# jiaw-z/DKT-Stereo

Measured on AMD Instinct MI355X. Metric: stereo pairs/sec at 736x1248 D=192, 32 iters (RAFT-Stereo test_mode forward), higher is better.
Workload: dtype f32 io/accumulate; convolution products = 3x fp16-split MFMA (22-bit operands); lookup / correlation exact fp32

## Files before the change

dkt_stereo_amd/csrc/conv_ws.h:

```cpp

static constexpr int conv_ws_group_first(int g) { return g < 5 ? g : g == 5 ? 5 : g < 10 ? g + 1 : g == 10 ? 11 : g + 2; }
static constexpr int conv_ws_group_units(int g) { return (g == 5 || g == 10) ? 2 : 1; }

static constexpr int conv_ws_rows_fed(int r, int nf) {
    int n = 0;
    for (int dy = 0; dy < 3; ++dy) n += (r - dy >= 0 && r - dy < nf) ? 1 : 0;
    return n;
}

typedef _Float16 ws_h2 __attribute__((ext_vector_type(2)));
typedef float ws_f2 __attribute__((ext_vector_type(2)));
__device__ __forceinline__ unsigned ws_bits(ws_h2 h) {
    union { ws_h2 h; unsigned u; } v;
    v.h = h;
    return v.u;
}

template <int NRM, int EPI>
__global__ __launch_bounds__(256, 1) void conv64_ws_kernel(ConvArgs a) {
    constexpr int HALO = 1;
    constexpr int NF = 4, WN = 2;
    constexpr int TR = NF * WN;
    constexpr int PR = TR + 2, PC = 34, NPP = PR * PC;
    constexpr int PITCH = 12;
    constexpr int PLANE = NPP * PITCH;
    constexpr int STAGE = 2 * PLANE;
    constexpr int NCH = 4;
    constexpr int NG = 16;
    constexpr int RB = 4;
    extern __shared__ __attribute__((aligned(16))) unsigned lds[];

    const int tid = threadIdx.x;
    const int lane = tid & 63, wave = tid >> 6;
    const int wm = wave & 1, wn = wave >> 1;
    const int li = lane & 31, kg = lane >> 5;
    const long HW = (long)a.H * a.W;
    const int tiles_h = a.tiles_xy / a.tiles_w;

    const int nblk = (int)gridDim.x;
    const int lb = (nblk % 8 == 0) ? ((int)blockIdx.x % 8) * (nblk / 8) + (int)blockIdx.x / 8 : (int)blockIdx.x;
    auto decode = [&](int t, int &th0, int &tw0, int &tb) {
        const int xy = t % a.tiles_xy;
        tb = t / a.tiles_xy;
        th0 = (xy % tiles_h) * TR;
        tw0 = (xy / tiles_h) * 32;
    };
    int h0, w0, b;
    int tile = lb;
    decode(tile, h0, w0, b);

    f16x8 Ahi[NCH * 9], Alo[NCH * 9];
    auto load_weights = [&]() {
        const long wlane = (long)(wm * 32 + li) * 16 + kg * 8;
#pragma unroll
        for (int c = 0; c < NCH; ++c)
#pragma unroll
            for (int tap = 0; tap < 9; ++tap) {
                const long off = ((long)tap * NCH + c) * (64 * 16) + wlane;
                Ahi[c * 9 + tap] = *(const f16x8 *)(a.whi + off);
                Alo[c * 9 + tap] = *(const f16x8 *)(a.wlo + off);
            }
#pragma unroll
        for (int i = 0; i < NCH * 9; ++i) {
            if (i < 24) {
                asm volatile("" : "+a"(Ahi[i]));
                asm volatile("" : "+a"(Alo[i]));
            } else {
                asm volatile("" : "+v"(Ahi[i]));
                asm volatile("" : "+v"(Alo[i]));
            }
        }
    };

    constexpr int SG = 2, PG = 2;
    constexpr int SIT = (NPP + 64 * PG - 1) / (64 * PG);
    constexpr int NSL = SIT * 4;
    const int swave = __builtin_amdgcn_readfirstlane(wave) % SG;
    const int spgrp = __builtin_amdgcn_readfirstlane(wave) / SG;
    unsigned spix[SIT];
    float sscale[SIT];
    float sreg[SIT][8];
    unsigned shw[SIT][4], slw[SIT][4];
    __amdgpu_buffer_rsrc_t srsrc;
    const unsigned plane_bytes = (unsigned)HW * 4u;
    float nmean[NRM ? 8 : 1], ninv[NRM ? 8 : 1];
    auto stage_tile = [&](int th0, int tw0) {
#pragma unroll
        for (int it = 0; it < SIT; ++it) {
            const int pp = lane + 64 * (it * PG + spgrp);
            const int pr = pp / PC, pc = pp - pr * PC;
            const int ih = th0 - HALO + pr, iw = tw0 - HALO + pc;
            const bool ok = pp < NPP && ih >= 0 && ih < a.H && iw >= 0 && iw < a.W;
            sscale[it] = ok ? a.in_scale : 0.0f;
            spix[it] = ok ? (unsigned)(ih * a.W + iw) * 4u : 0u;
        }
    };
    auto stage_select = [&](int tb, int chunk) {
        const int cb = chunk * 16 + 8 * swave;
        const float *sbase = a.src[0] + (long)tb * a.src_bs[0] + (long)cb * HW;
        const unsigned lo32 = __builtin_amdgcn_readfirstlane((unsigned)(size_t)sbase);
        const unsigned hi32 = __builtin_amdgcn_readfirstlane((unsigned)((size_t)sbase >> 32));
        srsrc = __builtin_amdgcn_make_buffer_rsrc((void *)(((size_t)hi32 << 32) | lo32), 0, (int)(8u * plane_bytes), 0x00020000);
        if (NRM) {
            const float *np = (const float *)(lds + 2 * STAGE + 8) + 2 * (tb * 64 + cb);
#pragma unroll
            for (int j = 0; j < (NRM ? 8 : 1); ++j) {
                nmean[j] = __int_as_float(__builtin_amdgcn_readfirstlane(__float_as_int(np[2 * j])));
                ninv[j] = __int_as_float(__builtin_amdgcn_readfirstlane(__float_as_int(np[2 * j + 1])));
            }
        }
    };
    auto stage_load = [&](int k0, int k1) {
#pragma unroll
        for (int k = k0; k < k1; ++k) {
            if (k >= NSL) break;
            const int it = k >> 2, q = k & 3;
#pragma unroll
            for (int jj = 0; jj < 2; ++jj) {
                const int j = 2 * q + jj;
                sreg[it][j] = __uint_as_float(__builtin_amdgcn_raw_buffer_load_b32(srsrc, spix[it], j * plane_bytes, 0));
            }
        }
    };
    auto stage_store = [&](unsigned *buf, int k0, int k1) {
#pragma unroll
        for (int k = k0; k < k1; ++k) {
            if (k >= NSL) break;
            const int it = k >> 2, q = k & 3;
            float u0 = sreg[it][2 * q], u1 = sreg[it][2 * q + 1];
            if (NRM) {
                u0 = dkt_relu(__fmul_rn(__fsub_rn(u0, nmean[(2 * q) % (NRM ? 8 : 1)]), ninv[(2 * q) % (NRM ? 8 : 1)]));
                u1 = dkt_relu(__fmul_rn(__fsub_rn(u1, nmean[(2 * q + 1) % (NRM ? 8 : 1)]), ninv[(2 * q + 1) % (NRM ? 8 : 1)]));
            }
            const ws_f2 xv = {u0 * sscale[it], u1 * sscale[it]};
            const ws_h2 hv = __builtin_convertvector(xv, ws_h2);
            const ws_f2 rv = {xv[0] - (float)hv[0], xv[1] - (float)hv[1]};
            const ws_h2 lv = __builtin_convertvector(rv, ws_h2);
            shw[it][q] = ws_bits(hv);
            slw[it][q] = ws_bits(lv);
            if (q == 3) {
                const int pp = lane + 64 * (it * PG + spgrp);
                unsigned *dst = pp < NPP ? buf + pp * PITCH + 4 * swave : lds + 2 * STAGE;
                *(uint4 *)dst = make_uint4(shw[it][0], shw[it][1], shw[it][2], shw[it][3]);
                *(uint4 *)(dst + (pp < NPP ? PLANE : 4)) = make_uint4(slw[it][0], slw[it][1], slw[it][2], slw[it][3]);
            }
        }
    };

    f32x16 acc[NF];
    auto zero_acc = [&]() {
#pragma unroll
        for (int n = 0; n < NF; ++n)
#pragma unroll
            for (int r = 0; r < 16; ++r) acc[n][r] = 0.0f;
    };
    zero_acc();

    f16x8 Bhi[RB], Blo[RB];
    auto loadB = [&](int slot, const unsigned *buf, int s) {
        const int dx = s / (NF + 2), r = s % (NF + 2);
        const int pp = (wn * NF + r) * PC + li + dx;
        const unsigned *pb = buf + pp * PITCH + kg * 4;
        Bhi[slot] = *(const f16x8 *)pb;
        Blo[slot] = *(const f16x8 *)(pb + PLANE);
    };
    auto mma = [&](const int c, const int s) {
        const int dx = s / (NF + 2), r = s % (NF + 2);
        const int slot = s % RB;
#pragma unroll
        for (int dy = 0; dy < 3; ++dy) {
            const int n = r - dy;
            if (n >= 0 && n < NF)
                acc[n] = __builtin_amdgcn_mfma_f32_32x32x16_f16(Ahi[c * 9 + dy * 3 + dx], Bhi[slot], acc[n], 0, 0, 0);
        }
#pragma unroll
        for (int dy = 0; dy < 3; ++dy) {
            const int n = r - dy;
            if (n >= 0 && n < NF)
                acc[n] = __builtin_amdgcn_mfma_f32_32x32x16_f16(Alo[c * 9 + dy * 3 + dx], Bhi[slot], acc[n], 0, 0, 0);
        }
#pragma unroll
        for (int dy = 0; dy < 3; ++dy) {
            const int n = r - dy;
            if (n >= 0 && n < NF)
                acc[n] = __builtin_amdgcn_mfma_f32_32x32x16_f16(Ahi[c * 9 + dy * 3 + dx], Blo[slot], acc[n], 0, 0, 0);
        }
    };

    auto mma_group = [&](const int c, const int g) {
#pragma unroll
        for (int pass = 0; pass < 3; ++pass)
#pragma unroll
            for (int u = conv_ws_group_first(g); u < conv_ws_group_first(g) + conv_ws_group_units(g); ++u) {
                const int dx = u / (NF + 2), r = u % (NF + 2);
#pragma unroll
                for (int dy = 0; dy < 3; ++dy) {
                    const int n = r - dy;
                    if (n >= 0 && n < NF) {
                        const int t = c * 9 + dy * 3 + dx;
                        acc[n] = __builtin_amdgcn_mfma_f32_32x32x16_f16(pass == 1 ? Alo[t] : Ahi[t], pass == 2 ? Blo[u % RB] : Bhi[u % RB],
                                                                        acc[n], 0, 0, 0);
                    }
                }
            }
    };

    auto wave_rsrc = [&](const float *base) {
        const unsigned lo32 = __builtin_amdgcn_readfirstlane((unsigned)(size_t)base);
        const unsigned hi32 = __builtin_amdgcn_readfirstlane((unsigned)((size_t)base >> 32));
        return __builtin_amdgcn_make_buffer_rsrc((void *)(((size_t)hi32 << 32) | lo32), 0, (int)(32u * plane_bytes), 0x00020000);
    };
    auto epilogue = [&]() {
        const int co_lane = wm * 32 + 4 * kg;
        float bv[16];
#pragma unroll
        for (int r = 0; r < 16; ++r) bv[r] = a.bias ? a.bias[co_lane + (r & 3) + 8 * (r >> 2)] : 0.0f;
        const auto orsrc = wave_rsrc(a.out + (long)b * a.out_bs + (long)(wm * 32) * HW);
        auto row_off = [&](int n, bool &ok) {
            const int oh = h0 + wn * NF + n, ow = w0 + li;
            ok = oh < a.H && ow < a.W;
            return ok ? (unsigned)(4 * kg) * plane_bytes + (unsigned)(oh * a.W + ow) * 4u : 0x80000000u;
        };
        if (EPI == 3) {
            const auto crsrc = wave_rsrc(a.e_c0 + (long)b * a.e_c0_bs + (long)(wm * 32) * HW);
            float gc[2][16];
            unsigned vo[NF];
            auto request = [&](int n) {
#pragma unroll
                for (int r = 0; r < 16; ++r)
                    gc[n & 1][r] = __uint_as_float(__builtin_amdgcn_raw_buffer_load_b32(crsrc, vo[n], ((r & 3) + 8 * (r >> 2)) * plane_bytes, 0));
            };
#pragma unroll
            for (int n = 0; n < NF; ++n) {
                bool ok;
                vo[n] = row_off(n, ok);
            }
            request(0);
            request(1);
#pragma unroll
            for (int n = 0; n < NF; ++n) {
                float o[16];
#pragma unroll
                for (int r = 0; r < 16; ++r) {
                    const float v = acc[n][r] * a.out_scale + bv[r];
                    o[r] = dkt_relu(__fadd_rn(gc[n & 1][r], a.relu ? dkt_relu(v) : v));
                }
                __builtin_amdgcn_sched_barrier(0);
                if (n + 2 < NF) request(n + 2);
                __builtin_amdgcn_sched_barrier(0);
#pragma unroll
                for (int r = 0; r < 16; ++r)
                    __builtin_amdgcn_raw_buffer_store_b32(__float_as_uint(o[r]), orsrc, vo[n], ((r & 3) + 8 * (r >> 2)) * plane_bytes, 0);
                __builtin_amdgcn_sched_barrier(0);
            }
            return;
        }
        float s1[EPI == 1 ? 16 : 1], s2[EPI == 1 ? 16 : 1];
#pragma unroll
        for (int i = 0; i < (EPI == 1 ? 16 : 1); ++i) s1[i] = s2[i] = 0.0f;
#pragma unroll
        for (int n = 0; n < NF; ++n) {
            bool ok;
            const unsigned vo = row_off(n, ok);
#pragma unroll
            for (int r = 0; r < 16; ++r) {
                float v = acc[n][r] * a.out_scale + bv[r];
                if (a.relu) v = dkt_relu(v);
                __builtin_amdgcn_raw_buffer_store_b32(__float_as_uint(v), orsrc, vo, ((r & 3) + 8 * (r >> 2)) * plane_bytes, 0);
                if (EPI == 1) {
                    v = ok ? v : 0.0f;
                    s1[r] = __fadd_rn(s1[r], v);
                    s2[r] = __fadd_rn(s2[r], __fmul_rn(v, v));
                }
            }
            __builtin_amdgcn_sched_barrier(0);
        }
        if (EPI == 1) {
#pragma unroll
            for (int i = 0; i < 16; ++i) {
                s1[i] = __fadd_rn(s1[i], __shfl_xor(s1[i], 16, 32));
                s2[i] = __fadd_rn(s2[i], __shfl_xor(s2[i], 16, 32));
            }
#pragma unroll
            for (int d = 8; d >= 1; d >>= 1) {
                const bool up = (li & d) != 0;
#pragma unroll
                for (int j = 0; j < d; ++j) {
                    const float k1 = up ? s1[j + d] : s1[j], g1 = up ? s1[j] : s1[j + d];
                    const float k2 = up ? s2[j + d] : s2[j], g2 = up ? s2[j] : s2[j + d];
                    s1[j] = __fadd_rn(k1, __shfl_xor(g1, d, 32));
                    s2[j] = __fadd_rn(k2, __shfl_xor(g2, d, 32));
                }
            }
            const int vi = li & 15;
            const int co = co_lane + (vi & 3) + 8 * (vi >> 2);
            const long e = (long)((h0 / TR) * a.tiles_w + w0 / 32) * WN + wn;
            if (li < 16) {
                float *p = a.stats_ws + (((long)b * a.tiles_xy * WN + e) * 64 + co) * 2;
                p[0] = s1[0];
                p[1] = s2[0];
            }
        }
    };

    if (NRM) {
        float *np = (float *)(lds + 2 * STAGE + 8);
        for (int i = tid; i < a.n_co * 128; i += 256) np[i] = a.in_norm[i];
        __syncthreads();
    }
    stage_tile(h0, w0);
    stage_select(b, 0);
    stage_load(0, NSL);
    stage_store(lds, 0, NSL);
    __builtin_amdgcn_sched_barrier(0);
    load_weights();
    __syncthreads();
    loadB(0, lds, 0);
    loadB(1, lds, 1);
    for (;;) {
        const int tn = tile + nblk;
        const bool have_next = tn < a.total_tiles;
        int nh0 = h0, nw0 = w0, nb = b;
        if (have_next) decode(tn, nh0, nw0, nb);
#pragma unroll
        for (int c = 0; c < NCH; ++c) {
            const unsigned *cur = lds + (c & 1) * STAGE;
            unsigned *nxt = lds + ((c + 1) & 1) * STAGE;
            if (c + 1 < NCH) {
                stage_select(b, c + 1);
            } else {
                stage_select(nb, 0);
                stage_tile(nh0, nw0);
            }
#pragma unroll
            for (int g = 0; g < NG; ++g) {
                if (g + 2 < NG) {
#pragma unroll
                    for (int u = conv_ws_group_first(g + 2); u < conv_ws_group_first(g + 2) + conv_ws_group_units(g + 2); ++u)
                        loadB(u % RB, cur, u);
                }
                if (g < 6) stage_load(2 * g, 2 * g + 2);
                else if (g == 9) stage_store(nxt, 0, 1);
                else if (g >= 10 && g < 15) stage_store(nxt, 2 * (g - 10) + 1, 2 * (g - 10) + 3);
                else if (g == 15) stage_store(nxt, 11, 12);
                mma_group(c, g);
                if (conv_ws_group_units(g) == 1 && conv_ws_rows_fed(conv_ws_group_first(g) % (NF + 2), NF) == 1) {
                    __builtin_amdgcn_sched_group_barrier(0x008, 3, 0);
                } else {
                    int nm = 0;
#pragma unroll
                    for (int u = conv_ws_group_first(g); u < conv_ws_group_first(g) + conv_ws_group_units(g); ++u)
                        nm += 3 * conv_ws_rows_fed(u % (NF + 2), NF);
#pragma unroll
                    for (int i = 0; i < nm; ++i) {
                        __builtin_amdgcn_sched_group_barrier(0x008, 1, 0);
                        __builtin_amdgcn_sched_group_barrier(0x320, 1, 0);
                        if (g >= 9) __builtin_amdgcn_sched_group_barrier(0x002, 4, 0);
                        else __builtin_amdgcn_sched_group_barrier(0x002, 2, 0);
                    }
                }
                __builtin_amdgcn_sched_barrier(0);
            }
            asm volatile("s_waitcnt lgkmcnt(0)" ::: "memory");
            __builtin_amdgcn_s_barrier();
            if (c + 1 < NCH) {
                loadB(0, nxt, 0);
                loadB(1, nxt, 1);
            }
        }
        epilogue();
        if (!have_next) break;
        tile = tn; h0 = nh0; w0 = nw0; b = nb;
        loadB(0, lds, 0);
        loadB(1, lds, 1);
        zero_acc();
    }
}

static int launch_conv_ws(ConvArgs a, int B, hipStream_t st) {
    constexpr int STAGE = 10 * 34 * 12 * 2;
    const size_t lds = ((size_t)2 * STAGE + 8) * sizeof(unsigned) + (a.in_norm ? (size_t)B * 512 : 0);
    static int ready[64] = {0};
    int dev = 0;
    (void)hipGetDevice(&dev);
    const int epi = a.epi == 3 ? 3 : (a.stats_ws ? 1 : 0);
    const void *kern = nullptr;
    if (a.in_norm) kern = epi == 3 ? (const void *)conv64_ws_kernel<1, 3> : epi == 1 ? (const void *)conv64_ws_kernel<1, 1> : (const void *)conv64_ws_kernel<1, 0>;
    else kern = epi == 3 ? (const void *)conv64_ws_kernel<0, 3> : epi == 1 ? (const void *)conv64_ws_kernel<0, 1> : (const void *)conv64_ws_kernel<0, 0>;
    if (!ready[dev & 63]) {
        const void *all[6] = {(const void *)conv64_ws_kernel<0, 0>, (const void *)conv64_ws_kernel<0, 1>, (const void *)conv64_ws_kernel<0, 3>,
                              (const void *)conv64_ws_kernel<1, 0>, (const void *)conv64_ws_kernel<1, 1>, (const void *)conv64_ws_kernel<1, 3>};
        for (int i = 0; i < 6; ++i) {
            hipError_t e = hipFuncSetAttribute(all[i], hipFuncAttributeMaxDynamicSharedMemorySize, (int)(((size_t)2 * STAGE + 8) * sizeof(unsigned)) + 64 * 512);
            if (e != hipSuccess) return (int)e;
        }
        int cus = 0;
        if (hipDeviceGetAttribute(&cus, hipDeviceAttributeMultiprocessorCount, dev) != hipSuccess || cus < 1) cus = 256;
        ready[dev & 63] = cus;
    }
    a.tiles_xy = a.tiles_w * ((a.H + 7) / 8);
    a.n_co = B;
    const long total = (long)a.tiles_xy * B;
    if (total > 0x7fffffffL) return DKT_E_SHAPE;
    a.total_tiles = (int)total;
    const long cap = ready[dev & 63];
    long nblk = total > cap ? cap : total;
    if (total > cap) {
        const long rounds = (total + cap - 1) / cap;
        const long need = ((total + rounds - 1) / rounds + 7) & ~7L;
        if (need < nblk) nblk = need;
    }
    void *params[1] = {(void *)&a};
    (void)hipLaunchKernel(kern, dim3((unsigned)nblk), dim3(256), params, lds, st);
    int rc = dkt_launch_status();
    if (rc == DKT_OK && a.stats_ws)
        rc = conv_stats_reduce(a.stats_ws, a.stats_part, B, a.Cout, (long)a.tiles_xy * 2, (long)a.H * a.W, a.out, a.out_bs, st);
    return rc;
}
```

Before: 33.11.

## Use 16x16x32 MFMA with swapped operands and vectorized epilogue stores in conv_ws

Adds a 16x16x32 MFMA variant of the 64-channel 3x3 conv kernel, used by default for the non-stats epilogues. It swaps operand roles so pixels feed the A slot and weights the B slot, and restructures the LDS staging layout into octet planes processed in two column phases per chunk. Because each lane now holds consecutive output pixels, the epilogue can emit 128-bit buffer stores and loads for residual input when the tile is fully in bounds. The aim is to cut strided scalar stores and possibly gain MFMA throughput. The cost is more complex scheduling, a new LDS layout and extra phase loops.

Result: no change. 33.10 (-0.0%).

```diff
diff --git a/dkt_stereo_amd/csrc/conv_ws.h b/dkt_stereo_amd/csrc/conv_ws.h
--- a/dkt_stereo_amd/csrc/conv_ws.h
+++ b/dkt_stereo_amd/csrc/conv_ws.h
@@ -1,3 +1,10 @@
+
+#ifdef CONV_WS_MFMA
+static constexpr int conv_ws_mfma(int, int) { return CONV_WS_MFMA; }
+#else
+static constexpr int conv_ws_mfma(int , int epi) { return epi == 1 ? 32 : 16; }
+#endif
+static constexpr int conv_ws_stage_words(int ms) { return ms == 16 ? 2 * 4 * 1408 : 2 * (10 * 34 + 1) * 12; }
 
 static constexpr int conv_ws_group_first(int g) { return g < 5 ? g : g == 5 ? 5 : g < 10 ? g + 1 : g == 10 ? 11 : g + 2; }
 static constexpr int conv_ws_group_units(int g) { return (g == 5 || g == 10) ? 2 : 1; }
@@ -10,6 +17,8 @@
 
 typedef _Float16 ws_h2 __attribute__((ext_vector_type(2)));
 typedef float ws_f2 __attribute__((ext_vector_type(2)));
+typedef float ws_f4 __attribute__((ext_vector_type(4)));
+typedef unsigned ws_u4 __attribute__((ext_vector_type(4)));
 __device__ __forceinline__ unsigned ws_bits(ws_h2 h) {
     union { ws_h2 h; unsigned u; } v;
     v.h = h;
@@ -18,22 +27,26 @@
 
 template <int NRM, int EPI>
 __global__ __launch_bounds__(256, 1) void conv64_ws_kernel(ConvArgs a) {
+    constexpr int MS = conv_ws_mfma(NRM, EPI);
     constexpr int HALO = 1;
     constexpr int NF = 4, WN = 2;
     constexpr int TR = NF * WN;
     constexpr int PR = TR + 2, PC = 34, NPP = PR * PC;
-    constexpr int PITCH = 12;
-    constexpr int PLANE = NPP * PITCH;
-    constexpr int STAGE = 2 * PLANE;
-    constexpr int NCH = 4;
+    constexpr int PITCH = MS == 16 ? 4 : 12;
+    constexpr int OCT = MS == 16 ? 1408 : 4;
+    constexpr int PLANE = MS == 16 ? 4 * OCT : (NPP + 1) * PITCH;
+    constexpr int STAGE = conv_ws_stage_words(MS);
+    constexpr int NCH = MS == 16 ? 2 : 4;
+    constexpr int NPH = MS == 16 ? 2 : 1;
     constexpr int NG = 16;
     constexpr int RB = 4;
+    constexpr int LSH = MS == 16 ? 4 : 5;
     extern __shared__ __attribute__((aligned(16))) unsigned lds[];
 
     const int tid = threadIdx.x;
     const int lane = tid & 63, wave = tid >> 6;
     const int wm = wave & 1, wn = wave >> 1;
-    const int li = lane & 31, kg = lane >> 5;
+    const int li = lane & (MS - 1), kg = lane >> LSH;
     const long HW = (long)a.H * a.W;
     const int tiles_h = a.tiles_xy / a.tiles_w;
 
@@ -49,25 +62,25 @@
     int tile = lb;
     decode(tile, h0, w0, b);
 
-    f16x8 Ahi[NCH * 9], Alo[NCH * 9];
+    f16x8 Whi[36], Wlo[36];
     auto load_weights = [&]() {
-        const long wlane = (long)(wm * 32 + li) * 16 + kg * 8;
-#pragma unroll
-        for (int c = 0; c < NCH; ++c)
-#pragma unroll
-            for (int tap = 0; tap < 9; ++tap) {
-                const long off = ((long)tap * NCH + c) * (64 * 16) + wlane;
-                Ahi[c * 9 + tap] = *(const f16x8 *)(a.whi + off);
-                Alo[c * 9 + tap] = *(const f16x8 *)(a.wlo + off);
-            }
-#pragma unroll
-        for (int i = 0; i < NCH * 9; ++i) {
+#pragma unroll
+        for (int i = 0; i < 36; ++i) {
+            const int h = MS == 16 ? i & 1 : 0, ct = MS == 16 ? i >> 1 : i;
+            const int c = ct / 9, tap = ct % 9;
+            const int ci16 = MS == 16 ? 2 * c + (kg >> 1) : c;
+            const long off = ((long)tap * 4 + ci16) * (64 * 16) + (long)(wm * 32 + 16 * h + li) * 16 + (MS == 16 ? kg & 1 : kg) * 8;
+            Whi[i] = *(const f16x8 *)(a.whi + off);
+            Wlo[i] = *(const f16x8 *)(a.wlo + off);
+        }
+#pragma unroll
+        for (int i = 0; i < 36; ++i) {
             if (i < 24) {
-                asm volatile("" : "+a"(Ahi[i]));
-                asm volatile("" : "+a"(Alo[i]));
+                asm volatile("" : "+a"(Whi[i]));
+                asm volatile("" : "+a"(Wlo[i]));
             } else {
-                asm volatile("" : "+v"(Ahi[i]));
-                asm volatile("" : "+v"(Alo[i]));
+                asm volatile("" : "+v"(Whi[i]));
+                asm volatile("" : "+v"(Wlo[i]));
             }
         }
     };
@@ -78,6 +91,12 @@
     const int swave = __builtin_amdgcn_readfirstlane(wave) % SG;
     const int spgrp = __builtin_amdgcn_readfirstlane(wave) / SG;
     unsigned spix[SIT];
+    unsigned sdst[SIT];
+#pragma unroll
+    for (int it = 0; it < SIT; ++it) {
+        const int pp = lane + 64 * (it * PG + spgrp);
+        sdst[it] = (unsigned)((pp < NPP ? pp : NPP) * PITCH);
+    }
     float sscale[SIT];
     float sreg[SIT][8];
     unsigned shw[SIT][4], slw[SIT][4];
@@ -95,14 +114,14 @@
             spix[it] = ok ? (unsigned)(ih * a.W + iw) * 4u : 0u;
         }
     };
-    auto stage_select = [&](int tb, int chunk) {
-        const int cb = chunk * 16 + 8 * swave;
+    auto stage_select = [&](int tb, int grp) {
+        const int cb = grp * 16 + 8 * swave;
         const float *sbase = a.src[0] + (long)tb * a.src_bs[0] + (long)cb * HW;
         const unsigned lo32 = __builtin_amdgcn_readfirstlane((unsigned)(size_t)sbase);
         const unsigned hi32 = __builtin_amdgcn_readfirstlane((unsigned)((size_t)sbase >> 32));
         srsrc = __builtin_amdgcn_make_buffer_rsrc((void *)(((size_t)hi32 << 32) | lo32), 0, (int)(8u * plane_bytes), 0x00020000);
         if (NRM) {
-            const float *np = (const float *)(lds + 2 * STAGE + 8) + 2 * (tb * 64 + cb);
+            const float *np = (const float *)(lds + 2 * STAGE) + 2 * (tb * 64 + cb);
 #pragma unroll
             for (int j = 0; j < (NRM ? 8 : 1); ++j) {
                 nmean[j] = __int_as_float(__builtin_amdgcn_readfirstlane(__float_as_int(np[2 * j])));
@@ -122,7 +141,7 @@
             }
         }
     };
-    auto stage_store = [&](unsigned *buf, int k0, int k1) {
+    auto stage_store = [&](unsigned *buf, const int grp, int k0, int k1) {
 #pragma unroll
         for (int k = k0; k < k1; ++k) {
             if (k >= NSL) break;
@@ -139,55 +158,43 @@
             shw[it][q] = ws_bits(hv);
             slw[it][q] = ws_bits(lv);
             if (q == 3) {
-                const int pp = lane + 64 * (it * PG + spgrp);
-                unsigned *dst = pp < NPP ? buf + pp * PITCH + 4 * swave : lds + 2 * STAGE;
+                const int oct = MS == 16 ? 2 * (grp & 1) + swave : swave;
+                unsigned *dst = buf + sdst[it] + oct * OCT;
                 *(uint4 *)dst = make_uint4(shw[it][0], shw[it][1], shw[it][2], shw[it][3]);
-                *(uint4 *)(dst + (pp < NPP ? PLANE : 4)) = make_uint4(slw[it][0], slw[it][1], slw[it][2], slw[it][3]);
-            }
-        }
-    };
-
-    f32x16 acc[NF];
+                *(uint4 *)(dst + PLANE) = make_uint4(slw[it][0], slw[it][1], slw[it][2], slw[it][3]);
+            }
+        }
+    };
+
+    ws_f4 acc16[MS == 16 ? 2 : 1][NF][2];
+    f32x16 acc32[NF];
     auto zero_acc = [&]() {
 #pragma unroll
-        for (int n = 0; n < NF; ++n)
-#pragma unroll
-            for (int r = 0; r < 16; ++r) acc[n][r] = 0.0f;
+        for (int n = 0; n < NF; ++n) {
+            if (MS == 16) {
+#pragma unroll
+                for (int i = 0; i < 4; ++i)
+#pragma unroll
+                    for (int r = 0; r < 4; ++r) acc16[(i >> 1) % (MS == 16 ? 2 : 1)][n][i & 1][r] = 0.0f;
+            } else {
+#pragma unroll
+                for (int r = 0; r < 16; ++r) acc32[n][r] = 0.0f;
+            }
+        }
     };
     zero_acc();
 
-    f16x8 Bhi[RB], Blo[RB];
-    auto loadB = [&](int slot, const unsigned *buf, int s) {
-        const int dx = s / (NF + 2), r = s % (NF + 2);
-        const int pp = (wn * NF + r) * PC + li + dx;
-        const unsigned *pb = buf + pp * PITCH + kg * 4;
-        Bhi[slot] = *(const f16x8 *)pb;
-        Blo[slot] = *(const f16x8 *)(pb + PLANE);
-    };
-    auto mma = [&](const int c, const int s) {
-        const int dx = s / (NF + 2), r = s % (NF + 2);
-        const int slot = s % RB;
-#pragma unroll
-        for (int dy = 0; dy < 3; ++dy) {
-            const int n = r - dy;
-            if (n >= 0 && n < NF)
-                acc[n] = __builtin_amdgcn_mfma_f32_32x32x16_f16(Ahi[c * 9 + dy * 3 + dx], Bhi[slot], acc[n], 0, 0, 0);
-        }
-#pragma unroll
-        for (int dy = 0; dy < 3; ++dy) {
-            const int n = r - dy;
-            if (n >= 0 && n < NF)
-                acc[n] = __builtin_amdgcn_mfma_f32_32x32x16_f16(Alo[c * 9 + dy * 3 + dx], Bhi[slot], acc[n], 0, 0, 0);
-        }
-#pragma unroll
-        for (int dy = 0; dy < 3; ++dy) {
-            const int n = r - dy;
-            if (n >= 0 && n < NF)
-                acc[n] = __builtin_amdgcn_mfma_f32_32x32x16_f16(Ahi[c * 9 + dy * 3 + dx], Blo[slot], acc[n], 0, 0, 0);
-        }
-    };
-
-    auto mma_group = [&](const int c, const int g) {
+    f16x8 Fhi[RB], Flo[RB];
+    const unsigned rbase = (unsigned)((wn * NF * PC + li) * PITCH + kg * OCT);
+    auto loadF = [&](int slot, const unsigned *buf, const int ph, const int u) {
+        const int dx = u / (NF + 2), r = u % (NF + 2);
+        const int pc = r * PC + 16 * ph + dx;
+        const unsigned *pb = buf + rbase + pc * PITCH;
+        Fhi[slot] = *(const f16x8 *)pb;
+        Flo[slot] = *(const f16x8 *)(pb + PLANE);
+    };
+
+    auto mma_group = [&](const int c, const int ph, const int g) {
 #pragma unroll
         for (int pass = 0; pass < 3; ++pass)
 #pragma unroll
@@ -198,8 +205,15 @@
                     const int n = r - dy;
                     if (n >= 0 && n < NF) {
                         const int t = c * 9 + dy * 3 + dx;
-                        acc[n] = __builtin_amdgcn_mfma_f32_32x32x16_f16(pass == 1 ? Alo[t] : Ahi[t], pass == 2 ? Blo[u % RB] : Bhi[u % RB],
-                                                                        acc[n], 0, 0, 0);
+                        const f16x8 x = pass == 2 ? Flo[u % RB] : Fhi[u % RB];
+                        if (MS == 16) {
+#pragma unroll
+                            for (int h = 0; h < 2; ++h)
+                                acc16[h % (MS == 16 ? 2 : 1)][n][ph] = __builtin_amdgcn_mfma_f32_16x16x32_f16(
+                                    x, pass == 1 ? Wlo[(2 * t + h) % 36] : Whi[(2 * t + h) % 36], acc16[h % (MS == 16 ? 2 : 1)][n][ph], 0, 0, 0);
+                        } else {
+                            acc32[n] = __builtin_amdgcn_mfma_f32_32x32x16_f16(x, pass == 1 ? Wlo[t % 36] : Whi[t % 36], acc32[n], 0, 0, 0);
+                        }
                     }
                 }
             }
@@ -210,113 +224,148 @@
         const unsigned hi32 = __builtin_amdgcn_readfirstlane((unsigned)((size_t)base >> 32));
         return __builtin_amdgcn_make_buffer_rsrc((void *)(((size_t)hi32 << 32) | lo32), 0, (int)(32u * plane_bytes), 0x00020000);
     };
-    auto epilogue = [&]() {
-        const int co_lane = wm * 32 + 4 * kg;
-        float bv[16];
-#pragma unroll
-        for (int r = 0; r < 16; ++r) bv[r] = a.bias ? a.bias[co_lane + (r & 3) + 8 * (r >> 2)] : 0.0f;
+    auto epilogue = [&](auto wide_c) {
+        constexpr bool WIDE = decltype(wide_c)::value;
+        constexpr int NQ = 4, NH = MS == 16 ? 2 : 1;
+        auto qh = [](int q) { return MS == 16 ? q >> 1 : 0; };
+        auto qpx = [](int q) { return MS == 16 ? 16 * (q & 1) : 8 * q; };
+        auto val = [&](int n, int q, int j) { return MS == 16 ? acc16[qh(q) % NH][n][q & 1][j] : acc32[n][4 * q + j]; };
+        int lane_e = lane;
+        asm volatile("" : "+v"(lane_e));
+        const int li = lane_e & (MS - 1), kg = lane_e >> LSH;
+        const int co_lane = wm * 32 + li;
+        float bv[NH];
+#pragma unroll
+        for (int h = 0; h < NH; ++h) bv[h] = a.bias ? a.bias[co_lane + 16 * h] : 0.0f;
         const auto orsrc = wave_rsrc(a.out + (long)b * a.out_bs + (long)(wm * 32) * HW);
-        auto row_off = [&](int n, bool &ok) {
-            const int oh = h0 + wn * NF + n, ow = w0 + li;
-            ok = oh < a.H && ow < a.W;
-            return ok ? (unsigned)(4 * kg) * plane_bytes + (unsigned)(oh * a.W + ow) * 4u : 0x80000000u;
+        unsigned vo[NF];
+        const int ow = w0 + 4 * kg;
+#pragma unroll
+        for (int n = 0; n < NF; ++n) {
+            const int oh = h0 + wn * NF + n;
+            vo[n] = oh < a.H ? (unsigned)li * plane_bytes + (unsigned)(oh * a.W + ow) * 4u : 0x80000000u;
+        }
+        auto q_soff = [&](int q) { return (unsigned)(16 * qh(q)) * plane_bytes + (unsigned)(qpx(q) * 4); };
+        const int left = a.W - ow;
+        auto q_voff = [&](int n, int q, int j) {
+            int lf = left;
+            if (!WIDE) asm volatile("" : "+v"(lf));
+            return qpx(q) + j < lf ? vo[n] : 0x80000000u;
+        };
+        auto store_run = [&](int n, int q, const float (&o)[4]) {
+            if (WIDE) {
+                const ws_u4 v = {__float_as_uint(o[0]), __float_as_uint(o[1]), __float_as_uint(o[2]), __float_as_uint(o[3])};
+                __builtin_amdgcn_raw_buffer_store_b128(v, orsrc, q_voff(n, q, 0), q_soff(q), 0);
+            } else {
+#pragma unroll
+                for (int j = 0; j < 4; ++j)
+                    __builtin_amdgcn_raw_buffer_store_b32(__float_as_uint(o[j]), orsrc, q_voff(n, q, j), q_soff(q) + 4 * j, 0);
+            }
         };
         if (EPI == 3) {
             const auto crsrc = wave_rsrc(a.e_c0 + (long)b * a.e_c0_bs + (long)(wm * 32) * HW);
-            float gc[2][16];
-            unsigned vo[NF];
+            float gc[2][NQ][4];
             auto request = [&](int n) {
 #pragma unroll
-                for (int r = 0; r < 16; ++r)
-                    gc[n & 1][r] = __uint_as_float(__builtin_amdgcn_raw_buffer_load_b32(crsrc, vo[n], ((r & 3) + 8 * (r >> 2)) * plane_bytes, 0));
+                for (int q = 0; q < NQ; ++q) {
+                    if (WIDE) {
+                        const ws_u4 v = __builtin_amdgcn_raw_buffer_load_b128(crsrc, q_voff(n, q, 0), q_soff(q), 0);
+#pragma unroll
+                        for (int j = 0; j < 4; ++j) gc[n & 1][q][j] = __uint_as_float(v[j]);
+                    } else {
+#pragma unroll
+                        for (int j = 0; j < 4; ++j)
+                            gc[n & 1][q][j] = __uint_as_float(__builtin_amdgcn_raw_buffer_load_b32(crsrc, q_voff(n, q, j), q_soff(q) + 4 * j, 0));
+                    }
+                }
             };
-#pragma unroll
-            for (int n = 0; n < NF; ++n) {
-                bool ok;
-                vo[n] = row_off(n, ok);
-            }
             request(0);
             request(1);
 #pragma unroll
             for (int n = 0; n < NF; ++n) {
-                float o[16];
-#pragma unroll
-                for (int r = 0; r < 16; ++r) {
-                    const float v = acc[n][r] * a.out_scale + bv[r];
-                    o[r] = dkt_relu(__fadd_rn(gc[n & 1][r], a.relu ? dkt_relu(v) : v));
-                }
+                float o[NQ][4];
+#pragma unroll
+                for (int q = 0; q < NQ; ++q)
+#pragma unroll
+                    for (int j = 0; j < 4; ++j) {
+                        const float v = val(n, q, j) * a.out_scale + bv[qh(q) % NH];
+                        o[q][j] = dkt_relu(__fadd_rn(gc[n & 1][q][j], a.relu ? dkt_relu(v) : v));
+                    }
                 __builtin_amdgcn_sched_barrier(0);
                 if (n + 2 < NF) request(n + 2);
                 __builtin_amdgcn_sched_barrier(0);
 #pragma unroll
-                for (int r = 0; r < 16; ++r)
-                    __builtin_amdgcn_raw_buffer_store_b32(__float_as_uint(o[r]), orsrc, vo[n], ((r & 3) + 8 * (r >> 2)) * plane_bytes, 0);
+                for (int q = 0; q < NQ; ++q) store_run(n, q, o[q]);
                 __builtin_amdgcn_sched_barrier(0);
             }
             return;
         }
-        float s1[EPI == 1 ? 16 : 1], s2[EPI == 1 ? 16 : 1];
-#pragma unroll
-        for (int i = 0; i < (EPI == 1 ? 16 : 1); ++i) s1[i] = s2[i] = 0.0f;
+        float s1[NH], s2[NH];
+#pragma unroll
+        for (int h = 0; h < NH; ++h) s1[h] = s2[h] = 0.0f;
 #pragma unroll
         for (int n = 0; n < NF; ++n) {
-            bool ok;
-            const unsigned vo = row_off(n, ok);
-#pragma unroll
-            for (int r = 0; r < 16; ++r) {
-                float v = acc[n][r] * a.out_scale + bv[r];
-                if (a.relu) v = dkt_relu(v);
-                __builtin_amdgcn_raw_buffer_store_b32(__float_as_uint(v), orsrc, vo, ((r & 3) + 8 * (r >> 2)) * plane_bytes, 0);
+#pragma unroll
+            for (int q = 0; q < NQ; ++q) {
+                float o[4];
+#pragma unroll
+                for (int j = 0; j < 4; ++j) {
+                    const float v = val(n, q, j) * a.out_scale + bv[qh(q) % NH];
+                    o[j] = a.relu ? dkt_relu(v) : v;
+                }
+                store_run(n, q, o);
                 if (EPI == 1) {
-                    v = ok ? v : 0.0f;
-                    s1[r] = __fadd_rn(s1[r], v);
-                    s2[r] = __fadd_rn(s2[r], __fmul_rn(v, v));
+                    float m[4];
+#pragma unroll
+                    for (int j = 0; j < 4; ++j) m[j] = q_voff(n, q, WIDE ? 0 : j) != 0x80000000u ? o[j] : 0.0f;
+                    s1[qh(q) % NH] = __fadd_rn(s1[qh(q) % NH], __fadd_rn(__fadd_rn(m[0], m[1]), __fadd_rn(m[2], m[3])));
+                    s2[qh(q) % NH] = __fadd_rn(s2[qh(q) % NH], __fadd_rn(__fadd_rn(__fmul_rn(m[0], m[0]), __fmul_rn(m[1], m[1])),
+                                                                         __fadd_rn(__fmul_rn(m[2], m[2]), __fmul_rn(m[3], m[3]))));
                 }
             }
             __builtin_amdgcn_sched_barrier(0);
         }
         if (EPI == 1) {
-#pragma unroll
-            for (int i = 0; i < 16; ++i) {
-                s1[i] = __fadd_rn(s1[i], __shfl_xor(s1[i], 16, 32));
-                s2[i] = __fadd_rn(s2[i], __shfl_xor(s2[i], 16, 32));
-            }
-#pragma unroll
-            for (int d = 8; d >= 1; d >>= 1) {
-                const bool up = (li & d) != 0;
-#pragma unroll
-                for (int j = 0; j < d; ++j) {
-                    const float k1 = up ? s1[j + d] : s1[j], g1 = up ? s1[j] : s1[j + d];
-                    const float k2 = up ? s2[j + d] : s2[j], g2 = up ? s2[j] : s2[j + d];
-                    s1[j] = __fadd_rn(k1, __shfl_xor(g1, d, 32));
-                    s2[j] = __fadd_rn(k2, __shfl_xor(g2, d, 32));
-                }
-            }
-            const int vi = li & 15;
-            const int co = co_lane + (vi & 3) + 8 * (vi >> 2);
             const long e = (long)((h0 / TR) * a.tiles_w + w0 / 32) * WN + wn;
-            if (li < 16) {
-                float *p = a.stats_ws + (((long)b * a.tiles_xy * WN + e) * 64 + co) * 2;
-                p[0] = s1[0];
-                p[1] = s2[0];
-            }
-        }
+#pragma unroll
+            for (int h = 0; h < NH; ++h) {
+#pragma unroll
+                for (int d = MS; d < 64; d <<= 1) {
+                    s1[h] = __fadd_rn(s1[h], __shfl_xor(s1[h], d, 64));
+                    s2[h] = __fadd_rn(s2[h], __shfl_xor(s2[h], d, 64));
+                }
+                if (kg == 0) {
+                    float *p = a.stats_ws + (((long)b * a.tiles_xy * WN + e) * 64 + co_lane + 16 * h) * 2;
+                    p[0] = s1[h];
+                    p[1] = s2[h];
+                }
+            }
+        }
+    };
+    auto run_epilogue = [&]() {
+        bool wide = (a.W & 3) == 0 && (((size_t)(a.out + (long)b * a.out_bs)) & 15) == 0;
+        if (EPI == 3) wide = wide && (((size_t)(a.e_c0 + (long)b * a.e_c0_bs)) & 15) == 0;
+        if (wide) epilogue(std::true_type());
+        else epilogue(std::false_type());
     };
 
     if (NRM) {
-        float *np = (float *)(lds + 2 * STAGE + 8);
+        float *np = (float *)(lds + 2 * STAGE);
         for (int i = tid; i < a.n_co * 128; i += 256) np[i] = a.in_norm[i];
         __syncthreads();
     }
     stage_tile(h0, w0);
-    stage_select(b, 0);
-    stage_load(0, NSL);
-    stage_store(lds, 0, NSL);
+#pragma unroll
+    for (int grp = 0; grp < NPH; ++grp) {
+        stage_select(b, grp);
+        stage_load(0, NSL);
+        stage_store(lds, grp, 0, NSL);
+    }
     __builtin_amdgcn_sched_barrier(0);
     load_weights();
     __syncthreads();
-    loadB(0, lds, 0);
-    loadB(1, lds, 1);
+    loadF(0, lds, 0, 0);
+    loadF(1, lds, 0, 1);
     for (;;) {
         const int tn = tile + nblk;
         const bool have_next = tn < a.total_tiles;
@@ -326,72 +375,83 @@
         for (int c = 0; c < NCH; ++c) {
             const unsigned *cur = lds + (c & 1) * STAGE;
             unsigned *nxt = lds + ((c + 1) & 1) * STAGE;
-            if (c + 1 < NCH) {
-                stage_select(b, c + 1);
-            } else {
-                stage_select(nb, 0);
-                stage_tile(nh0, nw0);
-            }
-#pragma unroll
-            for (int g = 0; g < NG; ++g) {
-                if (g + 2 < NG) {
-#pragma unroll
-                    for (int u = conv_ws_group_first(g + 2); u < conv_ws_group_first(g + 2) + conv_ws_group_units(g + 2); ++u)
-                        loadB(u % RB, cur, u);
-                }
-                if (g < 6) stage_load(2 * g, 2 * g + 2);
-                else if (g == 9) stage_store(nxt, 0, 1);
-                else if (g >= 10 && g < 15) stage_store(nxt, 2 * (g - 10) + 1, 2 * (g - 10) + 3);
-                else if (g == 15) stage_store(nxt, 11, 12);
-                mma_group(c, g);
-                if (conv_ws_group_units(g) == 1 && conv_ws_rows_fed(conv_ws_group_first(g) % (NF + 2), NF) == 1) {
-                    __builtin_amdgcn_sched_group_barrier(0x008, 3, 0);
+#pragma unroll
+            for (int ph = 0; ph < NPH; ++ph) {
+                const int sg = (c + 1) * NPH + ph;
+                if (sg < 4) {
+                    stage_select(b, sg);
                 } else {
-                    int nm = 0;
-#pragma unroll
-                    for (int u = conv_ws_group_first(g); u < conv_ws_group_first(g) + conv_ws_group_units(g); ++u)
-                        nm += 3 * conv_ws_rows_fed(u % (NF + 2), NF);
-#pragma unroll
-                    for (int i = 0; i < nm; ++i) {
-                        __builtin_amdgcn_sched_group_barrier(0x008, 1, 0);
-                        __builtin_amdgcn_sched_group_barrier(0x320, 1, 0);
-                        if (g >= 9) __builtin_amdgcn_sched_group_barrier(0x002, 4, 0);
-                        else __builtin_amdgcn_sched_group_barrier(0x002, 2, 0);
+                    stage_select(nb, sg - 4);
+                    if (sg == 4) stage_tile(nh0, nw0);
+                }
+#pragma unroll
+                for (int g = 0; g < NG; ++g) {
+                    if (g + 2 < NG) {
+#pragma unroll
+                        for (int u = conv_ws_group_first(g + 2); u < conv_ws_group_first(g + 2) + conv_ws_group_units(g + 2); ++u)
+                            loadF(u % RB, cur, ph, u);
                     }
-                }
-                __builtin_amdgcn_sched_barrier(0);
-            }
-            asm volatile("s_waitcnt lgkmcnt(0)" ::: "memory");
-            __builtin_amdgcn_s_barrier();
-            if (c + 1 < NCH) {
-                loadB(0, nxt, 0);
-                loadB(1, nxt, 1);
-            }
-        }
-        epilogue();
+                    if (g < 6) stage_load(2 * g, 2 * g + 2);
+                    else if (g == 9) stage_store(nxt, sg, 0, 1);
+                    else if (g >= 10 && g < 15) stage_store(nxt, sg, 2 * (g - 10) + 1, 2 * (g - 10) + 3);
+                    else if (g == 15) stage_store(nxt, sg, 11, 12);
+                    mma_group(c, ph, g);
+                    constexpr int PER = MS == 16 ? 2 : 1;
+                    if (conv_ws_group_units(g) == 1 && conv_ws_rows_fed(conv_ws_group_first(g) % (NF + 2), NF) == 1) {
+                        if (PER == 2) __builtin_amdgcn_sched_group_barrier(0x008, 6, 0);
+                        else __builtin_amdgcn_sched_group_barrier(0x008, 3, 0);
+                    } else {
+                        int nm = 0;
+#pragma unroll
+                        for (int u = conv_ws_group_first(g); u < conv_ws_group_first(g) + conv_ws_group_units(g); ++u)
+                            nm += 3 * PER * conv_ws_rows_fed(u % (NF + 2), NF);
+#pragma unroll
+                        for (int i = 0; i < nm; ++i) {
+                            __builtin_amdgcn_sched_group_barrier(0x008, 1, 0);
+                            if (i % PER == 0) __builtin_amdgcn_sched_group_barrier(0x320, 1, 0);
+                            if ((g >= 9 ? 4 : 2) / PER == 4) __builtin_amdgcn_sched_group_barrier(0x002, 4, 0);
+                            else if ((g >= 9 ? 4 : 2) / PER == 2) __builtin_amdgcn_sched_group_barrier(0x002, 2, 0);
+                            else __builtin_amdgcn_sched_group_barrier(0x002, 1, 0);
+                        }
+                    }
+                    __builtin_amdgcn_sched_barrier(0);
+                }
+                if (ph + 1 == NPH) {
+                    asm volatile("s_waitcnt lgkmcnt(0)" ::: "memory");
+                    __builtin_amdgcn_s_barrier();
+                }
+                if (ph + 1 < NPH) {
+                    loadF(0, cur, ph + 1, 0);
+                    loadF(1, cur, ph + 1, 1);
+                } else if (c + 1 < NCH) {
+                    loadF(0, nxt, 0, 0);
+                    loadF(1, nxt, 0, 1);
+                }
+            }
+        }
+        run_epilogue();
         if (!have_next) break;
         tile = tn; h0 = nh0; w0 = nw0; b = nb;
-        loadB(0, lds, 0);
-        loadB(1, lds, 1);
+        loadF(0, lds, 0, 0);
+        loadF(1, lds, 0, 1);
         zero_acc();
     }
 }
 
 static int launch_conv_ws(ConvArgs a, int B, hipStream_t st) {
-    constexpr int STAGE = 10 * 34 * 12 * 2;
-    const size_t lds = ((size_t)2 * STAGE + 8) * sizeof(unsigned) + (a.in_norm ? (size_t)B * 512 : 0);
     static int ready[64] = {0};
     int dev = 0;
     (void)hipGetDevice(&dev);
     const int epi = a.epi == 3 ? 3 : (a.stats_ws ? 1 : 0);
-    const void *kern = nullptr;
-    if (a.in_norm) kern = epi == 3 ? (const void *)conv64_ws_kernel<1, 3> : epi == 1 ? (const void *)conv64_ws_kernel<1, 1> : (const void *)conv64_ws_kernel<1, 0>;
-    else kern = epi == 3 ? (const void *)conv64_ws_kernel<0, 3> : epi == 1 ? (const void *)conv64_ws_kernel<0, 1> : (const void *)conv64_ws_kernel<0, 0>;
+    const struct { const void *kern; int stage; } all[6] = {
+        {(const void *)conv64_ws_kernel<0, 0>, conv_ws_stage_words(conv_ws_mfma(0, 0))}, {(const void *)conv64_ws_kernel<0, 1>, conv_ws_stage_words(conv_ws_mfma(0, 1))},
+        {(const void *)conv64_ws_kernel<0, 3>, conv_ws_stage_words(conv_ws_mfma(0, 3))}, {(const void *)conv64_ws_kernel<1, 0>, conv_ws_stage_words(conv_ws_mfma(1, 0))},
+        {(const void *)conv64_ws_kernel<1, 1>, conv_ws_stage_words(conv_ws_mfma(1, 1))}, {(const void *)conv64_ws_kernel<1, 3>, conv_ws_stage_words(conv_ws_mfma(1, 3))}};
+    const int which = (a.in_norm ? 3 : 0) + (epi == 3 ? 2 : epi);
+    const size_t lds = (size_t)2 * all[which].stage * sizeof(unsigned) + (a.in_norm ? (size_t)B * 512 : 0);
     if (!ready[dev & 63]) {
-        const void *all[6] = {(const void *)conv64_ws_kernel<0, 0>, (const void *)conv64_ws_kernel<0, 1>, (const void *)conv64_ws_kernel<0, 3>,
-                              (const void *)conv64_ws_kernel<1, 0>, (const void *)conv64_ws_kernel<1, 1>, (const void *)conv64_ws_kernel<1, 3>};
         for (int i = 0; i < 6; ++i) {
-            hipError_t e = hipFuncSetAttribute(all[i], hipFuncAttributeMaxDynamicSharedMemorySize, (int)(((size_t)2 * STAGE + 8) * sizeof(unsigned)) + 64 * 512);
+            hipError_t e = hipFuncSetAttribute(all[i].kern, hipFuncAttributeMaxDynamicSharedMemorySize, (int)((size_t)2 * all[i].stage * sizeof(unsigned)) + 64 * 512);
             if (e != hipSuccess) return (int)e;
         }
         int cus = 0;
@@ -411,7 +471,7 @@
         if (need < nblk) nblk = need;
     }
     void *params[1] = {(void *)&a};
-    (void)hipLaunchKernel(kern, dim3((unsigned)nblk), dim3(256), params, lds, st);
+    (void)hipLaunchKernel(all[which].kern, dim3((unsigned)nblk), dim3(256), params, lds, st);
     int rc = dkt_launch_status();
     if (rc == DKT_OK && a.stats_ws)
         rc = conv_stats_reduce(a.stats_ws, a.stats_part, B, a.Cout, (long)a.tiles_xy * 2, (long)a.H * a.W, a.out, a.out_bs, st);
```
